# janelia-flyem/flypylib

Measured on AMD Instinct MI355X. Metric: inference Mvoxels/sec, vgg_like (rf 18, 22^3 coarse -> 88^3 per reference tile), synthetic EM uint8 volume, higher is better.
Workload: dtype f16s; 1 GPU; the 520^3 volume of BASELINE.json's metric (configs[0]'s substack size) per GPU: vgg_like inference, 520x520x520 synthetic uint8 volume, reference tile lattice 102^3 (pitch 88), u8 in / f32 out resident in HBM; tile_in=102, executor=vgg_split_f16, parallelism=z-slab tile sharding x1, no collective, device=AMD Radeon Graphics (gfx950:sramecc+:xnack-)

## Files before the change

flypylib_amd/csrc/vgg_plan.h:

```cpp
#pragma once
#include <algorithm>
#include <cstdint>
#include <vector>

struct VggSlab {
  int64_t VZ, VY, VX;
  int64_t fz_hi;
  int64_t cz_lo, cz_hi;
  int CY, CX;
  bool empty;
};

static inline VggSlab vgg_slab(const int64_t dims[3], const std::vector<int32_t> &origins_z,
                               int32_t out_sz_z, int32_t zb, int32_t ze, int off) {
  VggSlab s = {};
  s.VZ = dims[0] - 2 * off; s.VY = dims[1] - 2 * off; s.VX = dims[2] - 2 * off;
  s.empty = s.VZ <= 0 || s.VY <= 0 || s.VX <= 0 || zb >= ze;
  if (s.empty) return s;
  const int64_t fz_lo = (int64_t)origins_z[zb] - off;
  s.fz_hi = std::min<int64_t>((int64_t)origins_z[ze - 1] - off + out_sz_z, s.VZ);
  s.cz_lo = fz_lo / 4; s.cz_hi = (s.fz_hi + 3) / 4;
  s.CY = (int)((s.VY + 3) / 4); s.CX = (int)((s.VX + 3) / 4);
  return s;
}

struct VggPyramid {
  int P2, P1;
  explicit VggPyramid(int64_t C) : P2((int)C + 2), P1(2 * P2 + 2) {}
};
struct Vgg2Pyramid {
  int Q, T3, H;
  explicit Vgg2Pyramid(int64_t C) : Q((int)C + 2), T3(2 * Q + 2), H(T3 + 2) {}
};

static inline int64_t vgg_chunk_rows(int64_t budget_bytes, int64_t bytes_per_fine_row,
                                     int fixed_rows, int64_t span, int64_t cap = 0) {
  int64_t c = std::max<int64_t>(4, (budget_bytes / bytes_per_fine_row - fixed_rows) / 2);
  c = std::min<int64_t>(c, span);
  c = (c + 3) / 4 * 4;
  return cap ? std::min<int64_t>(c, cap) : c;
}

static inline int64_t vgg_split_max_p1_rows(int P1Y, int P1X, int tile_z) {
  return ((int64_t)1 << 32) / 16 / ((int64_t)P1Y * P1X) - (tile_z + 2);
}
static inline int64_t vgg_split_chunk_cap(int64_t max_rows) {
  return std::max<int64_t>(4, ((max_rows - VggPyramid(0).P1) / 2) / 4 * 4);
}

enum { MID_INTERIOR = 0, MID_XCOL = 1, MID_ZLAYER = 2 };

struct MidGeo {
  int BZ, BY, BX;
  int ZS;
  constexpr int TZ() const { return BZ + 2; }
  constexpr int TY() const { return BY + 2; }
  constexpr int TX() const { return BX + 2; }
  constexpr int slots() const { return (TZ() - 1) * ZS + TY() * TX(); }
  constexpr int slot(int tz, int ty, int tx) const { return tz * ZS + ty * TX() + tx; }
};
constexpr MidGeo mid_geo(int o) {
  return o == MID_XCOL ? MidGeo{8, 16, 4, 108} : o == MID_ZLAYER ? MidGeo{4, 8, 16, 182} : MidGeo{8, 4, 16, 118};
}

struct MidVox { int z, y, x; };
constexpr MidVox mid_voxel(int o, int wave, int sub, int c) {
  return o == MID_XCOL     ? MidVox{2 * (wave >> 1) + (sub >> 1), c, 2 * (wave & 1) + (sub & 1)}
         : o == MID_ZLAYER ? MidVox{2 * (wave >> 2) + (sub >> 1), 2 * (wave & 3) + (sub & 1), c}
                           : MidVox{2 * (wave >> 1) + (sub >> 1), 2 * (wave & 1) + (sub & 1), c};
}
constexpr MidVox mid_slot_voxel(const MidGeo &g, int s) {
  const int tz = s / g.ZS < g.TZ() ? s / g.ZS : g.TZ() - 1;
  const int rem = s - tz * g.ZS < g.TY() * g.TX() ? s - tz * g.ZS : g.TY() * g.TX() - 1;
  return MidVox{tz, rem / g.TX(), rem % g.TX()};
}
constexpr int mid_tap_slot(const MidGeo &g, int tap) { return g.slot(tap / 9, (tap / 3) % 3, tap % 3); }

struct MidWalk {
  int nbx, nby, nbz;
  int z0, x0;
  constexpr int64_t blocks() const { return (int64_t)nbx * nby * nbz; }
};
struct MidPlan { MidWalk w[3]; };

static inline MidPlan vgg_mid_plan(int Z, int Y, int X, bool reorient) {
  auto cdiv = [](int a, int b) { return (a + b - 1) / b; };
  const MidGeo gi = mid_geo(MID_INTERIOR), gx = mid_geo(MID_XCOL), gz = mid_geo(MID_ZLAYER);
  MidPlan p = {};
  MidWalk &in = p.w[MID_INTERIOR], &xc = p.w[MID_XCOL], &zl = p.w[MID_ZLAYER];
  in = MidWalk{cdiv(2 * X, gi.BX), cdiv(2 * Y, gi.BY), cdiv(2 * Z, gi.BZ), 0, 0};
  if (!reorient) return p;
  const int live_x = 2 * X % gi.BX, live_z = 2 * Z % gi.BZ;
  if (live_x) {
    const MidWalk c = {cdiv(live_x, gx.BX), cdiv(2 * Y, gx.BY), cdiv(2 * Z, gx.BZ), 0, (in.nbx - 1) * gi.BX};
    if (c.blocks() < (int64_t)in.nby * in.nbz) { xc = c; --in.nbx; }
  }
  if (live_z && in.nbx) {
    const MidWalk c = {in.nbx, cdiv(2 * Y, gz.BY), cdiv(live_z, gz.BZ), (in.nbz - 1) * gi.BZ, 0};
    if (c.blocks() < (int64_t)in.nbx * in.nby) { zl = c; --in.nbz; }
  }
  return p;
}
```

flypylib_amd/csrc/vgg_split.hip:

```cpp
#define FPL_F16 1
#include <algorithm>
#include <cmath>
#include <initializer_list>

#include "fast_paths.h"
#include "mfma_util.h"
#include "pack_weights.h"
#include "vgg_plan.h"
#include <type_traits>
#include "vgg_split_lds.h"
#include "vgg_tiles.h"

namespace {

constexpr int CH = 48;
constexpr int CHP = 24, NPASS = CH / CHP;
constexpr int LO_OFF = CHP * 2;
constexpr int PASS_BYTES = 2 * LO_OFF;
constexpr int VOX = NPASS * PASS_BYTES;
constexpr int KS = (27 * CHP + 31) / 32;
constexpr int KTAB = (KS + 4) / 4 * 4;
constexpr int KTAB_BYTES = 4 * KTAB * 4;
static_assert(CHP % 8 == 0, "a lane's 8 k-slots stay inside one tap");

// ... 696 lines not shown
    for (int b = 0; b < 3; ++b) {
      const f32x4 sh = *reinterpret_cast<const f32x4 *>(a.shift3 + zero + 16 * b + 4 * g);
#pragma unroll
      for (int sub = 0; sub < 4; ++sub) acc[sub][b] = sh;
    }
    x8::conv_block(smem, ktab + 8 * g, td, origin(cur), origin(has_next ? nxt : cur), part, a.w3, vb,
                   sub_off, wave, lane, acc);
    asm volatile("" : "+s"(zero));
    const h16x8 *w4p = a.w4 + zero;
    f32x4 sh4[3];
#pragma unroll
    for (int b = 0; b < 3; ++b)
#pragma unroll
      for (int r = 0; r < 4; ++r) sh4[b][r] = a.shift4[zero + x8::out_channel(b, g, r)];
    h16x8 w4[3][4];
#pragma unroll
    for (int s = 0; s < 4; ++s)
#pragma unroll
      for (int b = 0; b < 3; ++b) w4[b][s] = w4p[(s * 3 + b) * 64 + lane];
    f32x4 pooled[3] = {{0.f, 0.f, 0.f, 0.f}, {0.f, 0.f, 0.f, 0.f}, {0.f, 0.f, 0.f, 0.f}};
    unsigned ovf = 0u;
#pragma unroll
    for (int sub = 0; sub < 4; ++sub) {
      const Frag2 h0 = pack_relu_split(acc[sub][0], acc[sub][1], ovf);
      const h16x8 hx = pack_relu_split_x(acc[sub][2], ovf);
#pragma unroll
      for (int b = 0; b < 3; ++b) {
        const f32x4 a4 = chain48(w4[b], h0, hx, sh4[b]);
#pragma unroll
        for (int r = 0; r < 4; ++r) pooled[b][r] = __builtin_fmaxf(pooled[b][r], a4[r]);
      }
    }
#pragma unroll
    for (int b = 0; b < 3; ++b)
#pragma unroll
      for (int r = 0; r < 4; ++r)
        pooled[b][r] = __builtin_fmaxf(pooled[b][r], __shfl_xor(pooled[b][r], 1));
    const int pz = 4 * cur.bz + pzl, py = 2 * cur.by + pyl, px = 8 * cur.bx + (c >> 1);
    const bool inside = pz < a.p2.Z && py < a.p2.Y && px < a.p2.X;
    if ((c & 1) == 0 && inside)
      x8::store12(a.p2, a.p2.vox(pz, py, px), g, pooled, ovf);
    ovf_all = pk_max_i16(ovf_all, inside ? ovf : 0u);
    if (!has_next) break;
    cur = nxt;
  }
  ovf_commit(ovf_all, a.flag, FPL_RANGE_MID);
}

static_assert(mid_geo(MID_INTERIOR).BZ == x8::BZ && mid_geo(MID_INTERIOR).BY == x8::BY &&
              mid_geo(MID_INTERIOR).BX == x8::BX && mid_geo(MID_INTERIOR).ZS == x8::ZS, "vgg_plan.h describes x8's block");
struct MidEdgeArgs {
  MidXArgs m;
  int z0, x0;
};

template <int O>
__global__ __launch_bounds__(64 * x8::WAVES, 2) void vggs_mid_pool_edge(MidEdgeArgs e) {
  constexpr MidGeo G = mid_geo(O);
  const MidXArgs &a = e.m;
  unsigned *ktab = reinterpret_cast<unsigned *>(smem + 2 * x8::BUF);
  const int tid = threadIdx.x, lane = tid & 63;
  const int wave = __builtin_amdgcn_readfirstlane(tid >> 6);
  const int c = lane & 15, g = lane >> 4;
  x8::ktab_init_oriented<O>(ktab, tid);
  const x8::TileDma td = x8::tile_dma_init_oriented<O>(wave, lane, a.p1.Y, a.p1.XP, (unsigned)a.p1.part_bytes());
  const int S = (int)gridDim.x >> 3, nbricks = a.walk.bricks();
  const int group = (int)blockIdx.x & 7, slot = (int)blockIdx.x >> 3;
  x8::Cursor cur;
  if (!x8::cursor_first(a.walk, nbricks, group, slot, S, cur)) return;
  const int64_t part = a.p1.part_bytes();
  auto origin = [&](const x8::Cursor &q) {
    return a.p1.p + a.p1.vox(e.z0 + G.BZ * q.bz, G.BY * q.by, e.x0 + G.BX * q.bx) * 16;
  };
  const MidVox v0 = mid_voxel(O, wave, 0, c);
  const unsigned vb = (unsigned)(G.slot(v0.z, v0.y, v0.x) * 16);
  auto sub_off = [](int sub) -> unsigned {
    const MidVox d = mid_voxel(O, 0, sub, 0);
    return (unsigned)(mid_geo(O).slot(d.z, d.y, d.x) * 16);
  };
  unsigned ovf_all = 0u;
  x8::prime(smem, td, origin(cur), part, a.w3, wave, lane);
  for (;;) {
    x8::Cursor nxt = cur;
    const bool has_next = x8::cursor_next(a.walk, slot, S, nxt);
    int zero = 0;
    asm volatile("" : "+s"(zero));
    f32x4 acc[4][3];
#pragma unroll
    for (int b = 0; b < 3; ++b) {
      const f32x4 sh = *reinterpret_cast<const f32x4 *>(a.shift3 + zero + 16 * b + 4 * g);
#pragma unroll
      for (int sub = 0; sub < 4; ++sub) acc[sub][b] = sh;
    }
    x8::conv_block(smem, ktab + 8 * g, td, origin(cur), origin(has_next ? nxt : cur), part, a.w3, vb,
                   sub_off, wave, lane, acc);
    asm volatile("" : "+s"(zero));
    const h16x8 *w4p = a.w4 + zero;
    f32x4 sh4[3];
#pragma unroll
    for (int b = 0; b < 3; ++b)
#pragma unroll
      for (int r = 0; r < 4; ++r) sh4[b][r] = a.shift4[zero + x8::out_channel(b, g, r)];
    h16x8 w4[3][4];
#pragma unroll
    for (int s = 0; s < 4; ++s)
#pragma unroll
      for (int b = 0; b < 3; ++b) w4[b][s] = w4p[(s * 3 + b) * 64 + lane];
    f32x4 pooled[3] = {{0.f, 0.f, 0.f, 0.f}, {0.f, 0.f, 0.f, 0.f}, {0.f, 0.f, 0.f, 0.f}};
    unsigned ovf = 0u;
#pragma unroll
    for (int sub = 0; sub < 4; ++sub) {
      const Frag2 h0 = pack_relu_split(acc[sub][0], acc[sub][1], ovf);
      const h16x8 hx = pack_relu_split_x(acc[sub][2], ovf);
#pragma unroll
      for (int b = 0; b < 3; ++b) {
        const f32x4 a4 = chain48(w4[b], h0, hx, sh4[b]);
#pragma unroll
        for (int r = 0; r < 4; ++r) pooled[b][r] = __builtin_fmaxf(pooled[b][r], a4[r]);
      }
    }
#pragma unroll
    for (int b = 0; b < 3; ++b)
#pragma unroll
      for (int r = 0; r < 4; ++r)
        pooled[b][r] = __builtin_fmaxf(pooled[b][r], __shfl_xor(pooled[b][r], 1));
    const int pz = (e.z0 + G.BZ * cur.bz + v0.z) >> 1, py = (G.BY * cur.by + v0.y) >> 1,
              px = (e.x0 + G.BX * cur.bx + v0.x) >> 1;
    const bool inside = pz < a.p2.Z && py < a.p2.Y && px < a.p2.X;
    if ((c & 1) == 0 && inside)
      x8::store12(a.p2, a.p2.vox(pz, py, px), g, pooled, ovf);
    ovf_all = pk_max_i16(ovf_all, inside ? ovf : 0u);
    if (!has_next) break;
    cur = nxt;
  }
  ovf_commit(ovf_all, a.flag, FPL_RANGE_MID);
}

constexpr int T_W7 = 3 * 6, T_W8 = 3;
__device__ __forceinline__ void head_chain(const f32x4 (&acc)[4][3], const unsigned char *w6p,
                                           const unsigned char *w7p, const unsigned char *w8p, const float *sh6p,
                                           const float *sh7p, float bias8, int lane, unsigned &ovf, float (&logit)[4]) {
  const int c = lane & 15, g = lane >> 4;
  auto frag = [&](const unsigned char *w, int part_, int nfrag, int f) {
    return *reinterpret_cast<const h16x8 *>(w + ((size_t)(part_ * nfrag + f) * 64 + lane) * 16);
  };
#pragma unroll
  for (int sp = 0; sp < 2; ++sp) {
    Frag2 h5[2];
    h16x8 h5x[2];
#pragma unroll
    for (int q = 0; q < 2; ++q) {
      h5[q] = pack_relu_split(acc[2 * sp + q][0], acc[2 * sp + q][1], ovf);
      h5x[q] = pack_relu_split_x(acc[2 * sp + q][2], ovf);
    }
    Frag2 h6[2][3];
#pragma unroll
    for (int s = 0; s < 3; ++s) {
      f32x4 a6[2][2];
#pragma unroll
      for (int bb = 0; bb < 2; ++bb) {
        const int b = 2 * s + bb;
        f32x4 sh;
#pragma unroll
        for (int r = 0; r < 4; ++r) sh[r] = sh6p[16 * b + 4 * g + r];
        h16x8 w6[4];
#pragma unroll
        for (int t = 0; t < 4; ++t) w6[t] = frag(w6p, 0, 0, t * 6 + b);
#pragma unroll
        for (int q = 0; q < 2; ++q) a6[q][bb] = chain48(w6, h5[q], h5x[q], sh);
      }
#pragma unroll
      for (int q = 0; q < 2; ++q) h6[q][s] = pack_relu_split(a6[q][0], a6[q][1], ovf);
    }
    f32x4 a8[2] = {{0.f, 0.f, 0.f, 0.f}, {0.f, 0.f, 0.f, 0.f}};
#pragma unroll
    for (int s = 0; s < 3; ++s) {
      f32x4 a7[2][2];
#pragma unroll
      for (int bb = 0; bb < 2; ++bb) {
        const int b = 2 * s + bb;
        f32x4 sh;
#pragma unroll
        for (int r = 0; r < 4; ++r) sh[r] = sh7p[16 * b + 4 * g + r];
#pragma unroll
// ... 417 lines not shown
    const fpl_op &op = prog->ops[conv_ops[l]];
    std::vector<float> scale(A + op.scale_off, A + op.scale_off + op.cout);
    st->off_w[l] = all.size() * sizeof(uint16_t);
    if (l == 0 && v2) {
      fpl_pack_stem2_split(A + op.w_off, scale.data(), op.cout, NPASS, CHP, &all);
    } else if (l == 0) {
      for (int part = 0; part < 2; ++part) {
        std::vector<uint16_t> f;
        fpl_pack_stem(A + op.w_off, scale.data(), op.cout, &f, part);
        all.insert(all.end(), f.begin(), f.end());
      }
    } else if (op.k == 3 && !v2) {
      fpl_pack_passes_split(A + op.w_off, scale.data(), op.cin, op.cout, x8::NQ, x8::CQ, x8::KQ, 0, &all);
    } else if (op.k == 3) {
      fpl_pack_passes_split(A + op.w_off, scale.data(), op.cin, op.cout, NPASS, CHP, KS,
                            v2 && l >= 1 && l <= 3, &all);
    } else if (op.cin == CH) {
      static const int blk[4][2] = {{0, 1}, {0, 1}, {2, 2}, {2, 2}};
      static const int part[4][2] = {{0, 0}, {1, 1}, {1, 0}, {0, 1}};
      std::vector<uint16_t> f;
      for (int s = 0; s < 4; ++s)
        fpl_pack_chain_step(A + op.w_off, scale.data(), op.cin, op.cout, mblocks[l], blk[s], part[s], &f,
                            op.cout == CH ? 2 : 0);
      all.insert(all.end(), f.begin(), f.end());
    } else {
      for (int part = 0; part < 2; ++part) {
        std::vector<uint16_t> f;
        fpl_pack_frags(A + op.w_off, scale.data(), 1, op.cin, op.cout, mblocks[l], ksteps[l],
                       SLOT_CHAIN, &f, false, part);
        all.insert(all.end(), f.begin(), f.end());
      }
    }
    st->off_s[l] = fpl_append_shifts(&shifts, A + op.shift_off, op.cout);
  }
  if (fpl_any_half_nonfinite(all))
    return fpl_fail_range(ctx, "a folded weight exceeds the IEEE-half range (65504); use precision "
                               "f32 (or 'auto') for this network");
  {
    const fpl_op &op0 = prog->ops[0];
    std::vector<float> sh48(48, 0.f);
    memcpy(sh48.data(), A + op0.shift_off, op0.cout * sizeof(float));
    st->xlim = (float)stem_input_limit(A, op0, A + op0.scale_off, sh48.data(), 1);
    if (!(st->xlim > 0.f))
      return fpl_fail_range(ctx, "the first layer's shift exceeds the IEEE-half range; use precision f32 "
                                 "(or 'auto') for this network");
  }
  st->bias8 = A[prog->ops[9].shift_off];
  FPL_TRY(fpl_upload_weight_set(ctx, all, shifts, &st->frags, &st->shifts));
  FPL_HIP(ctx, hipFuncSetAttribute((const void *)vggs_stem_pool<uint8_t>,
                                   hipFuncAttributeMaxDynamicSharedMemorySize, S_SMEM));
  FPL_HIP(ctx, hipFuncSetAttribute((const void *)vggs_stem_pool<float>,
                                   hipFuncAttributeMaxDynamicSharedMemorySize, S_SMEM));
  FPL_HIP(ctx, hipFuncSetAttribute((const void *)vggs_mid_pool,
                                   hipFuncAttributeMaxDynamicSharedMemorySize, x8::SMEM));
  FPL_HIP(ctx, hipFuncSetAttribute((const void *)vggs_mid_pool_edge<MID_XCOL>,
                                   hipFuncAttributeMaxDynamicSharedMemorySize, x8::SMEM));
  FPL_HIP(ctx, hipFuncSetAttribute((const void *)vggs_mid_pool_edge<MID_ZLAYER>,
                                   hipFuncAttributeMaxDynamicSharedMemorySize, x8::SMEM));
  FPL_HIP(ctx, hipFuncSetAttribute((const void *)vggs_c5_tail_p24,
                                   hipFuncAttributeMaxDynamicSharedMemorySize, M_SMEM));
  FPL_HIP(ctx, hipFuncSetAttribute((const void *)vggs_c5_tail,
                                   hipFuncAttributeMaxDynamicSharedMemorySize, x8::SMEM));
  FPL_HIP(ctx, hipFuncSetAttribute((const void *)vggs2_conv3<true, true, uint8_t>,
                                   hipFuncAttributeMaxDynamicSharedMemorySize, V2_SMEM));
  FPL_HIP(ctx, hipFuncSetAttribute((const void *)vggs2_conv3<true, true, float>,
                                   hipFuncAttributeMaxDynamicSharedMemorySize, V2_SMEM));
  FPL_HIP(ctx, hipFuncSetAttribute((const void *)vggs2_conv3<false, false, uint8_t>,
                                   hipFuncAttributeMaxDynamicSharedMemorySize, V2_SMEM));
  FPL_HIP(ctx, hipFuncSetAttribute((const void *)vggs2_conv3<false, true, uint8_t>,
                                   hipFuncAttributeMaxDynamicSharedMemorySize, V2_SMEM));
  st->version = prog->arena_version;
  st->int_valid = false;
  return 0;
}

int split_prepare_int(fpl_ctx *ctx, fpl_program *prog, SplitState *st, float mean, float sd) {
  if (st->int_valid && st->int_mean == mean && st->int_sd == sd) return 0;
  const fpl_op &op = prog->ops[0];
  const float *A = prog->arena_host.data();
  const double c0 = std::min(255.0, std::max(0.0, std::nearbyint((double)mean)));
  std::vector<float> scale(op.cout);
  st->shift1_int_host.assign(S_SHTAB, 0.f);
  const double k = (c0 - (double)mean) / (double)sd;
  for (int co = 0; co < op.cout; ++co) {
    scale[co] = (float)((double)A[op.scale_off + co] / (double)sd);
    for (int pz = 0; pz < 4; ++pz)
      for (int py = 0; py < 4; ++py)
        for (int px = 0; px < 4; ++px) {
          double sum = 0.0;
          for (int dz = 0; dz < 3 - pz; ++dz)
            for (int dy = 0; dy < 3 - py; ++dy)
              for (int dx = 0; dx < 3 - px; ++dx)
                sum += (double)A[op.w_off + (size_t)((dz * 3 + dy) * 3 + dx) * op.cout + co];
          st->shift1_int_host[(size_t)((pz * 4 + py) * 4 + px) * 48 + co] =
              (float)((double)A[op.shift_off + co] + k * sum * (double)A[op.scale_off + co]);
        }
  }
  st->w1_int_host.clear();
  if (fpl_vgg_variant(prog) == 2) {
    fpl_pack_stem2_split(A + op.w_off, scale.data(), op.cout, NPASS, CHP, &st->w1_int_host);
    st->w1_int_host.resize((size_t)2 * 6 * 512, 0);
  } else {
    for (int part = 0; part < 2; ++part) {
      std::vector<uint16_t> f;
      fpl_pack_stem(A + op.w_off, scale.data(), op.cout, &f, part);
      st->w1_int_host.insert(st->w1_int_host.end(), f.begin(), f.end());
// ... 83 lines not shown
      a.out = (unsigned char *)l3v; a.OZ = pz.T3; a.OY = py.T3; a.OX = px.T3;
      a.flag = flag;
      a.bg = BlockGrid{(int)ceil_div64(px.T3, 16), (int)ceil_div64(py.T3, 4), (int)ceil_div64(pz.T3, 4)};
      TimedLaunch tl(ctx, "vggs2_conv3");
      vggs2_conv3<false, false, uint8_t><<<brick_grid_size(a.bg), 256, V2_SMEM, stream>>>(a);
    }
    {
      V2SArgs a = {};
      a.in = (const unsigned char *)l3v; a.IZ = pz.T3; a.IY = py.T3; a.IX = px.T3;
      a.w = F + st->off_w[3]; a.shift = S + st->off_s[3];
      a.out = (unsigned char *)qv; a.OZ = pz.Q; a.OY = py.Q; a.OX = px.Q;
      a.flag = flag;
      a.bg = BlockGrid{(int)ceil_div64(px.Q, 8), (int)ceil_div64(py.Q, 2), (int)ceil_div64(pz.Q, 2)};
      TimedLaunch tl(ctx, "vggs2_conv3_pool");
      vggs2_conv3<false, true, uint8_t><<<brick_grid_size(a.bg), 256, V2_SMEM, stream>>>(a);
    }
    {
      TailSArgs a;
      a.p2 = (const unsigned char *)qv; a.P2Z = pz.Q; a.P2Y = py.Q; a.P2X = px.Q;
      a.w5 = F + st->off_w[4]; a.shift5 = S + st->off_s[4];
      a.CZ = CZ; a.CY = s.CY; a.CX = s.CX;
      a.w6 = F + st->off_w[5]; a.w7 = F + st->off_w[6]; a.w8 = F + st->off_w[7];
      a.shift6 = S + st->off_s[5]; a.shift7 = S + st->off_s[6]; a.bias8 = st->bias8;
      a.dst = dst; a.DY = SY; a.DX = SX; a.gz0 = c0;
      a.VZ = s.fz_hi; a.VY = s.VY; a.VX = s.VX; a.off = OFF;
      a.flag = flag;
      a.bg = BlockGrid{(int)ceil_div64(s.CX, 16), (int)ceil_div64(s.CY, 4), (int)ceil_div64(CZ, 4)};
      TimedLaunch tl(ctx, "vggs_c5_tail");
      vggs_c5_tail_p24<<<brick_grid_size(a.bg), 256, M_SMEM, stream>>>(a);
    }
    FPL_HIP(ctx, hipGetLastError());
  }
  return 0;
}

}

int fpl_split_infer_volume(fpl_ctx *ctx, fpl_program *prog, const void *src, int src_dtype,
                           float mean, float sd, const int64_t dims[3],
                           const std::vector<int32_t> origins[3], const int32_t out_sz[3],
                           int32_t zb, int32_t ze, float *dst) {
  SplitState *st;
  FPL_TRY(split_prepare(ctx, prog, &st));
  if (src_dtype == FPL_U8) FPL_TRY(split_prepare_int(ctx, prog, st, mean, sd));
  if (fpl_vgg_variant(prog) == 2)
    return split2_infer(ctx, st, src, src_dtype, mean, sd, dims, origins, out_sz, zb, ze, dst);
  hipStream_t stream = ctx->stream;
  const int64_t SZ = dims[0], SY = dims[1], SX = dims[2];
  const VggSlab s = vgg_slab(dims, origins[0], out_sz[0], zb, ze, 7);
  if (s.empty) return 0;
  const VggPyramid py(s.CY), px(s.CX);
  const char *edge_env = getenv("FPL_VGG_EDGE_BLOCKS");
  const int edge_blocks = edge_env ? atoi(edge_env) != 0 : 1;
  FPL_REQUIRE(ctx, (int64_t)S_TZ * SY * SX < ((int64_t)1 << 31),
              "vgg split path: a %lld x %lld plane is too large for the stem's 31-bit row "
              "offsets", (long long)SY, (long long)SX);
  const int64_t max_rows = vgg_split_max_p1_rows(py.P1, px.P1, x8::TZ);
  FPL_REQUIRE(ctx, max_rows >= 14,
              "vgg split path: a %lld x %lld plane is too large for the tile loader's 32-bit "
              "offsets", (long long)SY, (long long)SX);
  const int64_t cz_chunk = vgg_chunk_rows(fpl_vgg_scratch_budget(FPL_VGG_SCRATCH_DEFAULT),
                                          (int64_t)py.P1 * px.P1 * VOX, VggPyramid(0).P1, s.cz_hi - s.cz_lo,
                                          vgg_split_chunk_cap(max_rows));
  const VggPyramid pz_max(cz_chunk);
  DevTemp tmp(ctx);
  unsigned *flag;
  FPL_TRY(fpl_range_flag(ctx, &flag));
  x8::Tensor p1 = {nullptr, pz_max.P1, py.P1, px.P1, px.P1}, p2 = {nullptr, pz_max.P2, py.P2, px.P2, px.P2};
  void *p1v, *p2v;
  FPL_TRY(tmp.alloc((size_t)(p1.bytes() + p1.slack_bytes()), &p1v));
  FPL_TRY(tmp.alloc((size_t)(p2.bytes() + p2.slack_bytes()), &p2v));
  void *dumpv;
  FPL_TRY(tmp.alloc(256, &dumpv));
  const unsigned pgrid = (unsigned)std::max(8, ctx->n_cu / 8 * 8);
  const unsigned char *F = st->frags;
  const float *S = st->shifts;
  for (int64_t c0 = s.cz_lo; c0 < s.cz_hi; c0 += cz_chunk) {
    const int CZ = (int)std::min<int64_t>(cz_chunk, s.cz_hi - c0);
    const VggPyramid pz(CZ);
    p1 = x8::Tensor{(unsigned char *)p1v, pz.P1, py.P1, px.P1, px.P1};
    p2 = x8::Tensor{(unsigned char *)p2v, pz.P2, py.P2, px.P2, px.P2};
    FPL_HIP(ctx, hipMemsetAsync(p1.p + p1.bytes(), 0, (size_t)p1.slack_bytes(), stream));
    FPL_HIP(ctx, hipMemsetAsync(p2.p + p2.bytes(), 0, (size_t)p2.slack_bytes(), stream));
    {
      StemSArgs a;
      a.src = src; a.SZ = SZ; a.SY = SY; a.SX = SX; a.mean = mean; a.sd = sd;
      a.p1z0 = 2 * c0;
      a.z_hi = std::min<int64_t>(SZ, 4 * (c0 + CZ) + 14);
      a.w1 = (const h16x8 *)(F + st->off_w[0]);
      a.w2 = (const h16x8 *)(F + st->off_w[1]);
      a.shift1 = S + st->off_s[0]; a.shift2 = S + st->off_s[1];
      a.c0 = 0.f; a.shtab = nullptr;
      if (src_dtype == FPL_U8) {
        a.w1 = (const h16x8 *)st->w1_int; a.shtab = st->shift1_int;
        a.c0 = st->int_c0;
      }
      a.p1 = p1;
      a.flag = flag; a.xlim = st->xlim; a.dump = (unsigned char *)dumpv;
      a.nbx = (int)ceil_div64(px.P1, S_PX); a.nby = (int)ceil_div64(py.P1, S_PY);
      a.nbz = (int)ceil_div64(pz.P1, S_PZ);
      a.trim = edge_blocks;
      const unsigned grid = (unsigned)std::min<int64_t>((int64_t)a.nbx * a.nby * a.nbz,
                                                        (int64_t)ctx->n_cu);
      TimedLaunch tl(ctx, "vggs_stem_pool");
      if (src_dtype == FPL_U8)
        vggs_stem_pool<uint8_t><<<grid, 64 * S_WAVES, S_SMEM, stream>>>(a);
      else
        vggs_stem_pool<float><<<grid, 64 * S_WAVES, S_SMEM, stream>>>(a);
    }
    {
      MidXArgs a;
      a.p1 = p1;
      a.w3 = F + st->off_w[2];
      a.w4 = (const h16x8 *)(F + st->off_w[3]);
      a.shift3 = S + st->off_s[2]; a.shift4 = S + st->off_s[3];
      a.p2 = p2;
      a.flag = flag;
      const MidPlan mp = vgg_mid_plan(pz.P2, py.P2, px.P2, edge_blocks != 0);
      auto walk_of = [&](int o) { return x8::Walk{mp.w[o].nbx, mp.w[o].nby, mp.w[o].nbz}; };
      TimedLaunch tl(ctx, "vggs_mid_pool");
      if (mp.w[MID_INTERIOR].blocks()) {
        a.walk = walk_of(MID_INTERIOR);
        vggs_mid_pool<<<pgrid, 64 * x8::WAVES, x8::SMEM, stream>>>(a);
      }
      for (int o : {MID_XCOL, MID_ZLAYER}) {
        if (!mp.w[o].blocks()) continue;
        MidEdgeArgs e = {a, mp.w[o].z0, mp.w[o].x0};
        e.m.walk = walk_of(o);
        const unsigned egrid = (unsigned)std::min<int64_t>(pgrid, (mp.w[o].blocks() + 7) / 8 * 8);
        if (o == MID_XCOL)
          vggs_mid_pool_edge<MID_XCOL><<<egrid, 64 * x8::WAVES, x8::SMEM, stream>>>(e);
        else
          vggs_mid_pool_edge<MID_ZLAYER><<<egrid, 64 * x8::WAVES, x8::SMEM, stream>>>(e);
      }
    }
    {
      TailXArgs a;
      a.p2 = p2;
      a.w5 = F + st->off_w[4]; a.shift5 = S + st->off_s[4];
      a.CZ = CZ; a.CY = s.CY; a.CX = s.CX;
      a.w6 = F + st->off_w[5]; a.w7 = F + st->off_w[6]; a.w8 = F + st->off_w[7];
      a.shift6 = S + st->off_s[5]; a.shift7 = S + st->off_s[6]; a.bias8 = st->bias8;
      a.dst = dst; a.DY = SY; a.DX = SX; a.gz0 = c0;
      a.VZ = s.fz_hi; a.VY = s.VY; a.VX = s.VX; a.off = 7;
      a.flag = flag;
      a.walk = x8::Walk{(int)ceil_div64(s.CX, 16), (int)ceil_div64(s.CY, 4), (int)ceil_div64(CZ, 8)};
      TimedLaunch tl(ctx, "vggs_c5_tail");
      vggs_c5_tail<<<pgrid, 64 * x8::WAVES, x8::SMEM, stream>>>(a);
    }
    FPL_HIP(ctx, hipGetLastError());
  }
  return 0;
}
```

flypylib_amd/csrc/vgg_split_lds.h:

```cpp
#pragma once
#include "mfma_util.h"
#include "vgg_plan.h"
#include "vgg_tiles.h"

namespace x8 {

constexpr int CQ = 8, NQ = 6;
constexpr int KQ = 7;
constexpr int BZ = 8, BY = 4, BX = 16;
constexpr int TZ = BZ + 2, TY = BY + 2, TX = BX + 2;
constexpr int ZS = 118;
constexpr int PLANE = (TZ - 1) * ZS + TY * TX;
constexpr int CHUNKS = (2 * PLANE + 63) / 64;
constexpr int TILE_BYTES = CHUNKS * 1024;
constexpr int WFRAGS = KQ * 6;
constexpr int WBYTES = WFRAGS * 1024;
constexpr int BUF = TILE_BYTES + WBYTES;
constexpr int KTAB_BYTES = 4 * 8 * 4;
constexpr int SMEM = 2 * BUF + KTAB_BYTES;
constexpr int WAVES = 8;
constexpr int TCH = (CHUNKS + WAVES - 1) / WAVES;
constexpr int WCH = (WFRAGS + WAVES - 1) / WAVES;
static_assert((ZS - 2 * TX - 2) % 16 == 0 && (TX - 2) % 16 == 0, "conflict-free tap offsets");
static_assert(SMEM <= 160 * 1024, "one workgroup per CU");
// ... 206 lines not shown
};
__device__ __forceinline__ bool cursor_first(const Walk &w, int , int group, int slot, int S, Cursor &c) {
  const int total = w.nbx * w.nby * w.nbz, per = (total + 7) / 8;
  c.i = group * per + slot;
  c.iend = (group + 1) * per < total ? (group + 1) * per : total;
  if (c.i >= c.iend) return false;
  walk_decode(w, c.i, c.bx, c.by, c.bz);
  return true;
}
__device__ __forceinline__ bool cursor_next(const Walk &w, int , int S, Cursor &c) {
  c.i += S;
  if (c.i >= c.iend) return false;
  walk_decode(w, c.i, c.bx, c.by, c.bz);
  return true;
}

__host__ __device__ constexpr int out_channel(int b, int g, int r) { return b < 2 ? 8 * g + 4 * b + r : 32 + 4 * g + r; }
__device__ __forceinline__ void store12(const Tensor &t, int64_t vox, int g, const f32x4 (&v)[3], unsigned &ovf) {
  unsigned hi[6], lo[6];
#pragma unroll
  for (int b = 0; b < 3; ++b) {
    const Pair2 p0 = split_pk(v[b][0], v[b][1], ovf), p1 = split_pk(v[b][2], v[b][3], ovf);
    hi[2 * b] = p0.hi; hi[2 * b + 1] = p1.hi;
    lo[2 * b] = p0.lo; lo[2 * b + 1] = p1.lo;
  }
  const int64_t part = t.part_bytes();
  unsigned char *q = t.p + (int64_t)g * 2 * part + vox * 16;
  unsigned char *h = t.p + (int64_t)(4 + (g >> 1)) * 2 * part + vox * 16 + 8 * (g & 1);
  *reinterpret_cast<u32x4 *>(q) = u32x4{hi[0], hi[1], hi[2], hi[3]};
  *reinterpret_cast<u32x4 *>(q + part) = u32x4{lo[0], lo[1], lo[2], lo[3]};
  *reinterpret_cast<u32x2 *>(h) = u32x2{hi[4], hi[5]};
  *reinterpret_cast<u32x2 *>(h + part) = u32x2{lo[4], lo[5]};
}

__device__ __forceinline__ void store12_sel(const Tensor &t, int64_t vox, int g, const f32x4 (&v)[3],
                                            unsigned &ovf, bool valid, unsigned char *dump) {
  unsigned hi[6], lo[6], o2 = 0u;
#pragma unroll
  for (int b = 0; b < 3; ++b) {
    const Pair2 p0 = split_pk(v[b][0], v[b][1], o2), p1 = split_pk(v[b][2], v[b][3], o2);
    hi[2 * b] = p0.hi; hi[2 * b + 1] = p1.hi;
    lo[2 * b] = p0.lo; lo[2 * b + 1] = p1.lo;
  }
  ovf_note(ovf, valid ? o2 : 0u);
  const int64_t part = t.part_bytes();
  unsigned char *q = t.p + (int64_t)g * 2 * part + vox * 16;
  unsigned char *h = t.p + (int64_t)(4 + (g >> 1)) * 2 * part + vox * 16 + 8 * (g & 1);
  *reinterpret_cast<u32x4 *>(valid ? q : dump) = u32x4{hi[0], hi[1], hi[2], hi[3]};
  *reinterpret_cast<u32x4 *>(valid ? q + part : dump + 16) = u32x4{lo[0], lo[1], lo[2], lo[3]};
  *reinterpret_cast<u32x2 *>(valid ? h : dump + 32) = u32x2{hi[4], hi[5]};
  *reinterpret_cast<u32x2 *>(valid ? h + part : dump + 48) = u32x2{lo[4], lo[5]};
}

}
```

Baseline: 16190 Mvoxels/s.

## Add 8x8x16 y-doubled mid-pool block kernel with single weight buffer

```diff
diff --git a/flypylib_amd/csrc/vgg_plan.h b/flypylib_amd/csrc/vgg_plan.h
--- a/flypylib_amd/csrc/vgg_plan.h
+++ b/flypylib_amd/csrc/vgg_plan.h
@@ -48,7 +48,7 @@
   return std::max<int64_t>(4, ((max_rows - VggPyramid(0).P1) / 2) / 4 * 4);
 }
 
-enum { MID_INTERIOR = 0, MID_XCOL = 1, MID_ZLAYER = 2 };
+enum { MID_INTERIOR = 0, MID_XCOL = 1, MID_ZLAYER = 2, MID_Y8 = 3 };
 
 struct MidGeo {
   int BZ, BY, BX;
@@ -60,13 +60,18 @@
   constexpr int slot(int tz, int ty, int tx) const { return tz * ZS + ty * TX() + tx; }
 };
 constexpr MidGeo mid_geo(int o) {
-  return o == MID_XCOL ? MidGeo{8, 16, 4, 108} : o == MID_ZLAYER ? MidGeo{4, 8, 16, 182} : MidGeo{8, 4, 16, 118};
+  return o == MID_XCOL     ? MidGeo{8, 16, 4, 108}
+         : o == MID_ZLAYER ? MidGeo{4, 8, 16, 182}
+         : o == MID_Y8     ? MidGeo{8, 8, 16, 182}
+                           : MidGeo{8, 4, 16, 118};
 }
+constexpr int mid_subs(int o) { return o == MID_Y8 ? 8 : 4; }
 
 struct MidVox { int z, y, x; };
 constexpr MidVox mid_voxel(int o, int wave, int sub, int c) {
   return o == MID_XCOL     ? MidVox{2 * (wave >> 1) + (sub >> 1), c, 2 * (wave & 1) + (sub & 1)}
          : o == MID_ZLAYER ? MidVox{2 * (wave >> 2) + (sub >> 1), 2 * (wave & 3) + (sub & 1), c}
+         : o == MID_Y8     ? MidVox{2 * (wave >> 1) + ((sub >> 1) & 1), 4 * (wave & 1) + 2 * (sub >> 2) + (sub & 1), c}
                            : MidVox{2 * (wave >> 1) + (sub >> 1), 2 * (wave & 1) + (sub & 1), c};
 }
 constexpr MidVox mid_slot_voxel(const MidGeo &g, int s) {
@@ -75,6 +80,10 @@
   return MidVox{tz, rem / g.TX(), rem % g.TX()};
 }
 constexpr int mid_tap_slot(const MidGeo &g, int tap) { return g.slot(tap / 9, (tap / 3) % 3, tap % 3); }
+
+constexpr int MID_Y8_CHUNKS = (2 * mid_geo(MID_Y8).slots() + 63) / 64;
+constexpr int MID_Y8_ROUNDS = (MID_Y8_CHUNKS + 7) / 8;
+constexpr int mid_y8_chunk(int wave, int i) { return wave + 8 * i < MID_Y8_CHUNKS ? wave + 8 * i : -1; }
 
 struct MidWalk {
   int nbx, nby, nbz;
@@ -101,3 +110,22 @@
   }
   return p;
 }
+
+struct MidPlanY8 {
+  MidPlan p;
+  MidWalk y8;
+  int strip_y0;
+};
+
+static inline MidPlanY8 vgg_mid_plan_y8(int Z, int Y, int X, bool reorient, bool large) {
+  MidPlanY8 q = {vgg_mid_plan(Z, Y, X, reorient), MidWalk{}, 0};
+  MidWalk &in = q.p.w[MID_INTERIOR];
+  const MidGeo gi = mid_geo(MID_INTERIOR), g8 = mid_geo(MID_Y8);
+  const int rows8 = Y % 4 == 3 ? Y / 4 + 1 : Y / 4;
+  if (!large || !rows8 || !in.blocks()) return q;
+  q.y8 = MidWalk{in.nbx, rows8, in.nbz, 0, 0};
+  q.strip_y0 = rows8 * g8.BY;
+  in.nby = (2 * Y - q.strip_y0 + gi.BY - 1) / gi.BY;
+  if (in.nby <= 0) in = MidWalk{};
+  return q;
+}
diff --git a/flypylib_amd/csrc/vgg_split.hip b/flypylib_amd/csrc/vgg_split.hip
--- a/flypylib_amd/csrc/vgg_split.hip
+++ b/flypylib_amd/csrc/vgg_split.hip
@@ -772,6 +772,7 @@
 struct MidEdgeArgs {
   MidXArgs m;
   int z0, x0;
+  int y0;
 };
 
 template <int O>
@@ -790,7 +791,7 @@
   if (!x8::cursor_first(a.walk, nbricks, group, slot, S, cur)) return;
   const int64_t part = a.p1.part_bytes();
   auto origin = [&](const x8::Cursor &q) {
-    return a.p1.p + a.p1.vox(e.z0 + G.BZ * q.bz, G.BY * q.by, e.x0 + G.BX * q.bx) * 16;
+    return a.p1.p + a.p1.vox(e.z0 + G.BZ * q.bz, e.y0 + G.BY * q.by, e.x0 + G.BX * q.bx) * 16;
   };
   const MidVox v0 = mid_voxel(O, wave, 0, c);
   const unsigned vb = (unsigned)(G.slot(v0.z, v0.y, v0.x) * 16);
@@ -844,12 +845,92 @@
 #pragma unroll
       for (int r = 0; r < 4; ++r)
         pooled[b][r] = __builtin_fmaxf(pooled[b][r], __shfl_xor(pooled[b][r], 1));
-    const int pz = (e.z0 + G.BZ * cur.bz + v0.z) >> 1, py = (G.BY * cur.by + v0.y) >> 1,
+    const int pz = (e.z0 + G.BZ * cur.bz + v0.z) >> 1, py = (e.y0 + G.BY * cur.by + v0.y) >> 1,
               px = (e.x0 + G.BX * cur.bx + v0.x) >> 1;
     const bool inside = pz < a.p2.Z && py < a.p2.Y && px < a.p2.X;
     if ((c & 1) == 0 && inside)
       x8::store12(a.p2, a.p2.vox(pz, py, px), g, pooled, ovf);
     ovf_all = pk_max_i16(ovf_all, inside ? ovf : 0u);
+    if (!has_next) break;
+    cur = nxt;
+  }
+  ovf_commit(ovf_all, a.flag, FPL_RANGE_MID);
+}
+
+__global__ __launch_bounds__(64 * x8::WAVES, 2) void vggs_mid_pool_y8(MidXArgs a) {
+  namespace y8 = x8::y8;
+  constexpr MidGeo G = y8::G;
+  unsigned *ktab = reinterpret_cast<unsigned *>(smem + y8::KTAB_OFF);
+  const int tid = threadIdx.x, lane = tid & 63;
+  const int wave = __builtin_amdgcn_readfirstlane(tid >> 6);
+  const int c = lane & 15, g = lane >> 4;
+  y8::ktab_init(ktab, tid);
+  const y8::TileDma td = y8::tile_dma_init(wave, lane, a.p1.Y, a.p1.XP, (unsigned)a.p1.part_bytes());
+  const int S = (int)gridDim.x >> 3, nbricks = a.walk.bricks();
+  const int group = (int)blockIdx.x & 7, slot = (int)blockIdx.x >> 3;
+  x8::Cursor cur;
+  if (!x8::cursor_first(a.walk, nbricks, group, slot, S, cur)) return;
+  const int64_t part = a.p1.part_bytes();
+  auto origin = [&](const x8::Cursor &q) {
+    return a.p1.p + a.p1.vox(G.BZ * q.bz, G.BY * q.by, G.BX * q.bx) * 16;
+  };
+  const MidVox v0 = mid_voxel(MID_Y8, wave, 0, c);
+  const unsigned vb = (unsigned)(G.slot(v0.z, v0.y, v0.x) * 16);
+  unsigned ovf_all = 0u;
+  y8::prime(smem, td, origin(cur), a.w3, wave, lane);
+  for (;;) {
+    x8::Cursor nxt = cur;
+    const bool has_next = x8::cursor_next(a.walk, slot, S, nxt);
+    int zero = 0;
+    asm volatile("" : "+s"(zero));
+    f32x4 acc[y8::SUBS][3];
+#pragma unroll
+    for (int b = 0; b < 3; ++b) {
+      const f32x4 sh = *reinterpret_cast<const f32x4 *>(a.shift3 + zero + 16 * b + 4 * g);
+#pragma unroll
+      for (int sub = 0; sub < y8::SUBS; ++sub) acc[sub][b] = sh;
+    }
+    y8::conv_block(smem, ktab + 8 * g, td, origin(cur), origin(has_next ? nxt : cur), part, a.w3, vb, wave, lane,
+                   acc);
+    asm volatile("" : "+s"(zero));
+    const h16x8 *w4p = a.w4 + zero;
+    f32x4 sh4[3];
+#pragma unroll
+    for (int b = 0; b < 3; ++b)
+#pragma unroll
+      for (int r = 0; r < 4; ++r) sh4[b][r] = a.shift4[zero + x8::out_channel(b, g, r)];
+    h16x8 w4[3][4];
+#pragma unroll
+    for (int s = 0; s < 4; ++s)
+#pragma unroll
+      for (int b = 0; b < 3; ++b) w4[b][s] = w4p[(s * 3 + b) * 64 + lane];
+#pragma unroll
+    for (int win = 0; win < y8::SUBS / 4; ++win) {
+      f32x4 pooled[3] = {{0.f, 0.f, 0.f, 0.f}, {0.f, 0.f, 0.f, 0.f}, {0.f, 0.f, 0.f, 0.f}};
+      unsigned ovf = 0u;
+#pragma unroll
+      for (int sub = 4 * win; sub < 4 * win + 4; ++sub) {
+        const Frag2 h0 = pack_relu_split(acc[sub][0], acc[sub][1], ovf);
+        const h16x8 hx = pack_relu_split_x(acc[sub][2], ovf);
+#pragma unroll
+        for (int b = 0; b < 3; ++b) {
+          const f32x4 a4 = chain48(w4[b], h0, hx, sh4[b]);
+#pragma unroll
+          for (int r = 0; r < 4; ++r) pooled[b][r] = __builtin_fmaxf(pooled[b][r], a4[r]);
+        }
+      }
+#pragma unroll
+      for (int b = 0; b < 3; ++b)
+#pragma unroll
+        for (int r = 0; r < 4; ++r)
+          pooled[b][r] = __builtin_fmaxf(pooled[b][r], __shfl_xor(pooled[b][r], 1));
+      const MidVox vw = mid_voxel(MID_Y8, wave, 4 * win, c);
+      const int pz = (G.BZ * cur.bz + vw.z) >> 1, py = (G.BY * cur.by + vw.y) >> 1, px = (G.BX * cur.bx + vw.x) >> 1;
+      const bool inside = pz < a.p2.Z && py < a.p2.Y && px < a.p2.X;
+      if ((c & 1) == 0 && inside)
+        x8::store12(a.p2, a.p2.vox(pz, py, px), g, pooled, ovf);
+      ovf_all = pk_max_i16(ovf_all, inside ? ovf : 0u);
+    }
     if (!has_next) break;
     cur = nxt;
   }
@@ -1373,6 +1454,10 @@
   FPL_HIP(ctx, hipFuncSetAttribute((const void *)vggs_stem_pool<float>,
                                    hipFuncAttributeMaxDynamicSharedMemorySize, S_SMEM));
   FPL_HIP(ctx, hipFuncSetAttribute((const void *)vggs_mid_pool,
+                                   hipFuncAttributeMaxDynamicSharedMemorySize, x8::SMEM));
+  FPL_HIP(ctx, hipFuncSetAttribute((const void *)vggs_mid_pool_y8,
+                                   hipFuncAttributeMaxDynamicSharedMemorySize, x8::y8::SMEM));
+  FPL_HIP(ctx, hipFuncSetAttribute((const void *)vggs_mid_pool_edge<MID_INTERIOR>,
                                    hipFuncAttributeMaxDynamicSharedMemorySize, x8::SMEM));
   FPL_HIP(ctx, hipFuncSetAttribute((const void *)vggs_mid_pool_edge<MID_XCOL>,
                                    hipFuncAttributeMaxDynamicSharedMemorySize, x8::SMEM));
@@ -1562,6 +1647,8 @@
   const VggPyramid py(s.CY), px(s.CX);
   const char *edge_env = getenv("FPL_VGG_EDGE_BLOCKS");
   const int edge_blocks = edge_env ? atoi(edge_env) != 0 : 1;
+  const char *mid_env = getenv("FPL_VGG_MID_BLOCK");
+  const int mid_large = mid_env ? atoi(mid_env) != 0 : 1;
   FPL_REQUIRE(ctx, (int64_t)S_TZ * SY * SX < ((int64_t)1 << 31),
               "vgg split path: a %lld x %lld plane is too large for the stem's 31-bit row "
               "offsets", (long long)SY, (long long)SX);
@@ -1626,19 +1713,27 @@
       a.shift3 = S + st->off_s[2]; a.shift4 = S + st->off_s[3];
       a.p2 = p2;
       a.flag = flag;
-      const MidPlan mp = vgg_mid_plan(pz.P2, py.P2, px.P2, edge_blocks != 0);
-      auto walk_of = [&](int o) { return x8::Walk{mp.w[o].nbx, mp.w[o].nby, mp.w[o].nbz}; };
+      const MidPlanY8 mq = vgg_mid_plan_y8(pz.P2, py.P2, px.P2, edge_blocks != 0, mid_large != 0);
+      const MidPlan &mp = mq.p;
+      auto walk_of = [&](const MidWalk &w) { return x8::Walk{w.nbx, w.nby, w.nbz}; };
+      auto grid_of = [&](const MidWalk &w) { return (unsigned)std::min<int64_t>(pgrid, (w.blocks() + 7) / 8 * 8); };
       TimedLaunch tl(ctx, "vggs_mid_pool");
-      if (mp.w[MID_INTERIOR].blocks()) {
-        a.walk = walk_of(MID_INTERIOR);
+      if (mq.y8.blocks()) {
+        a.walk = walk_of(mq.y8);
+        vggs_mid_pool_y8<<<grid_of(mq.y8), 64 * x8::WAVES, x8::y8::SMEM, stream>>>(a);
+      }
+      if (mp.w[MID_INTERIOR].blocks() && !mq.strip_y0) {
+        a.walk = walk_of(mp.w[MID_INTERIOR]);
         vggs_mid_pool<<<pgrid, 64 * x8::WAVES, x8::SMEM, stream>>>(a);
       }
-      for (int o : {MID_XCOL, MID_ZLAYER}) {
-        if (!mp.w[o].blocks()) continue;
-        MidEdgeArgs e = {a, mp.w[o].z0, mp.w[o].x0};
-        e.m.walk = walk_of(o);
-        const unsigned egrid = (unsigned)std::min<int64_t>(pgrid, (mp.w[o].blocks() + 7) / 8 * 8);
-        if (o == MID_XCOL)
+      for (int o : {MID_INTERIOR, MID_XCOL, MID_ZLAYER}) {
+        if (!mp.w[o].blocks() || (o == MID_INTERIOR && !mq.strip_y0)) continue;
+        MidEdgeArgs e = {a, mp.w[o].z0, mp.w[o].x0, o == MID_INTERIOR ? mq.strip_y0 : 0};
+        e.m.walk = walk_of(mp.w[o]);
+        const unsigned egrid = grid_of(mp.w[o]);
+        if (o == MID_INTERIOR)
+          vggs_mid_pool_edge<MID_INTERIOR><<<egrid, 64 * x8::WAVES, x8::SMEM, stream>>>(e);
+        else if (o == MID_XCOL)
           vggs_mid_pool_edge<MID_XCOL><<<egrid, 64 * x8::WAVES, x8::SMEM, stream>>>(e);
         else
           vggs_mid_pool_edge<MID_ZLAYER><<<egrid, 64 * x8::WAVES, x8::SMEM, stream>>>(e);
diff --git a/flypylib_amd/csrc/vgg_split_lds.h b/flypylib_amd/csrc/vgg_split_lds.h
--- a/flypylib_amd/csrc/vgg_split_lds.h
+++ b/flypylib_amd/csrc/vgg_split_lds.h
@@ -282,4 +282,202 @@
   *reinterpret_cast<u32x2 *>(valid ? h + part : dump + 48) = u32x2{lo[4], lo[5]};
 }
 
-}
+namespace y8 {
+
+constexpr MidGeo G = mid_geo(MID_Y8);
+constexpr int SUBS = mid_subs(MID_Y8);
+constexpr int PLANE = G.slots();
+constexpr int CHUNKS = MID_Y8_CHUNKS;
+constexpr int TCH = MID_Y8_ROUNDS;
+constexpr int TILE_BYTES = CHUNKS * 1024;
+constexpr int WA = 4 * 6, WB = WFRAGS - WA;
+constexpr int W_OFF = 2 * TILE_BYTES;
+constexpr int KTAB_OFF = W_OFF + WBYTES;
+constexpr int SMEM = KTAB_OFF + KTAB_BYTES;
+static_assert(G.BZ == 8 && G.BY == 8 && G.BX == 16 && SUBS * WAVES * 16 == G.BZ * G.BY * G.BX, "");
+static_assert((G.ZS - 2 * G.TX() - 2) % 16 == 0 && (G.TX() - 2) % 16 == 0, "conflict-free tap offsets");
+static_assert(PLANE == 1818 && CHUNKS == 57 && TCH == 8 && SMEM == 159872 && SMEM <= 160 * 1024, "LDS budget");
+static_assert(WA % WAVES == 0 && WB <= 3 * WAVES, "weight chunk deal");
+
+struct TileDma {
+  unsigned off[TCH];
+};
+__device__ __forceinline__ TileDma tile_dma_init(int wave, int lane, int SY, int SX, unsigned part_bytes) {
+  TileDma d;
+#pragma unroll
+  for (int i = 0; i < TCH; ++i) {
+    int slot = 64 * (wave + WAVES * i) + lane;
+    slot = slot < 2 * PLANE ? slot : 2 * PLANE - 1;
+    const int part = slot >= PLANE;
+    const MidVox v = mid_slot_voxel(G, slot - part * PLANE);
+    d.off[i] = (unsigned)(((v.z * SY + v.y) * SX + v.x) * 16) + (part ? part_bytes : 0u);
+  }
+  return d;
+}
+
+__device__ __forceinline__ void ktab_init(unsigned *ktab, int tid) {
+  if (tid < 32) {
+    const int g = tid >> 3, s = tid & 7;
+    const int tap = 4 * s + g;
+    ktab[tid] = tap < 27 ? (unsigned)(mid_tap_slot(G, tap) * 16) : 0u;
+  }
+}
+
+__device__ __forceinline__ void dma_tile(const TileDma &d, int i, int wave, const unsigned char *org, unsigned char *tile) {
+  const int j = wave + WAVES * i;
+  if (i < TCH - 1 || j < CHUNKS) {
+    asm volatile("" : "+s"(org));
+    glds16(org + d.off[i], tile + j * 1024);
+  }
+}
+__device__ __forceinline__ void dma_weights(int first, int n, int k, int wave, int lane, const unsigned char *wpass,
+                                            unsigned char *wbuf) {
+  const int j = wave + WAVES * k;
+  if (j < n) {
+    const unsigned char *src = wpass + (first + j) * 1024;
+    asm volatile("" : "+s"(src));
+    glds16(src + (unsigned)lane * 16u, wbuf + (first + j) * 1024);
+  }
+}
+
+__device__ __forceinline__ void dma_step(int s, const TileDma &d, int wave, int lane, const unsigned char *wcur,
+                                         const unsigned char *wnxt, const unsigned char *org, unsigned char *tile,
+                                         unsigned char *wbuf) {
+  if (s == 0) {
+#pragma unroll
+    for (int k = 0; k < 3; ++k) dma_weights(WA, WB, k, wave, lane, wcur, wbuf);
+  } else if (s == 1 || s == 2) {
+#pragma unroll
+    for (int k = 0; k < 3; ++k) dma_tile(d, 3 * (s - 1) + k, wave, org, tile);
+  } else if (s == 3) {
+    dma_tile(d, 6, wave, org, tile);
+    dma_tile(d, 7, wave, org, tile);
+    dma_weights(0, WA, 0, wave, lane, wnxt, wbuf);
+  } else if (s == 4) {
+    dma_weights(0, WA, 1, wave, lane, wnxt, wbuf);
+    dma_weights(0, WA, 2, wave, lane, wnxt, wbuf);
+  }
+}
+
+__device__ __forceinline__ constexpr unsigned sub_off(int sub) {
+  return (unsigned)(G.slot(mid_voxel(MID_Y8, 0, sub, 0).z, mid_voxel(MID_Y8, 0, sub, 0).y, 0) * 16);
+}
+
+template <typename Issue>
+__device__ __forceinline__ void pass_kloop(const unsigned char *tile, const unsigned char *wbuf, const unsigned *ktab_g,
+                                           unsigned vb, Issue issue, int lane, f32x4 (&acc)[SUBS][3]) {
+  const unsigned char *wl = wbuf + lane * 16;
+  const u32x4 k0 = *reinterpret_cast<const u32x4 *>(ktab_g), k1 = *reinterpret_cast<const u32x4 *>(ktab_g + 4);
+  Frag2 ba[4], bb[4];
+  h16x8 w[6];
+#pragma unroll
+  for (int q = 0; q < 4; ++q) {
+    const unsigned char *p = tile + vb + k0[0] + sub_off(q);
+    ba[q].hi = *reinterpret_cast<const h16x8 *>(p);
+    ba[q].lo = *reinterpret_cast<const h16x8 *>(p + PLANE * 16);
+  }
+#pragma unroll
+  for (int f = 0; f < 6; ++f) w[f] = *reinterpret_cast<const h16x8 *>(wl + f * 1024);
+#pragma unroll
+  for (int s = 0; s < KQ; ++s) {
+    const unsigned kcur = s < 4 ? k0[s & 3] : k1[s & 3];
+    __builtin_amdgcn_sched_barrier(0);
+    __builtin_amdgcn_s_setprio(1);
+#pragma unroll
+    for (int q = 0; q < 4; ++q)
+#pragma unroll
+      for (int b = 0; b < 3; ++b) acc[q][b] = mfma16(w[3 + b], ba[q].hi, acc[q][b]);
+    __builtin_amdgcn_sched_barrier(0);
+#pragma unroll
+    for (int q = 0; q < 4; ++q) {
+      const unsigned char *p = tile + vb + kcur + sub_off(4 + q);
+      bb[q].hi = *reinterpret_cast<const h16x8 *>(p);
+      bb[q].lo = *reinterpret_cast<const h16x8 *>(p + PLANE * 16);
+    }
+    __builtin_amdgcn_sched_barrier(0);
+#pragma unroll
+    for (int q = 0; q < 4; ++q)
+#pragma unroll
+      for (int b = 0; b < 3; ++b) acc[q][b] = mfma16(w[b], ba[q].lo, acc[q][b]);
+    __builtin_amdgcn_sched_barrier(0);
+    issue(s);
+    __builtin_amdgcn_sched_barrier(0);
+#pragma unroll
+    for (int q = 0; q < 4; ++q)
+#pragma unroll
+      for (int b = 0; b < 3; ++b) acc[q][b] = mfma16(w[b], ba[q].hi, acc[q][b]);
+#pragma unroll
+    for (int q = 0; q < 4; ++q)
+#pragma unroll
+      for (int b = 0; b < 3; ++b) acc[4 + q][b] = mfma16(w[3 + b], bb[q].hi, acc[4 + q][b]);
+    __builtin_amdgcn_sched_barrier(0);
+    if (s + 1 < KQ) {
+      const unsigned knxt = s + 1 < 4 ? k0[(s + 1) & 3] : k1[(s + 1) & 3];
+#pragma unroll
+      for (int q = 0; q < 4; ++q) {
+        const unsigned char *p = tile + vb + knxt + sub_off(q);
+        ba[q].hi = *reinterpret_cast<const h16x8 *>(p);
+        ba[q].lo = *reinterpret_cast<const h16x8 *>(p + PLANE * 16);
+      }
+#pragma unroll
+      for (int f = 3; f < 6; ++f) w[f] = *reinterpret_cast<const h16x8 *>(wl + ((s + 1) * 6 + f) * 1024);
+    }
+    __builtin_amdgcn_sched_barrier(0);
+#pragma unroll
+    for (int q = 0; q < 4; ++q)
+#pragma unroll
+      for (int b = 0; b < 3; ++b) acc[4 + q][b] = mfma16(w[b], bb[q].lo, acc[4 + q][b]);
+#pragma unroll
+    for (int q = 0; q < 4; ++q)
+#pragma unroll
+      for (int b = 0; b < 3; ++b) acc[4 + q][b] = mfma16(w[b], bb[q].hi, acc[4 + q][b]);
+    __builtin_amdgcn_s_setprio(0);
+    __builtin_amdgcn_sched_barrier(0);
+    if (s + 1 < KQ) {
+#pragma unroll
+      for (int f = 0; f < 3; ++f) w[f] = *reinterpret_cast<const h16x8 *>(wl + ((s + 1) * 6 + f) * 1024);
+    }
+  }
+}
+
+__device__ __forceinline__ void conv_block(unsigned char *smem, const unsigned *ktab_g, const TileDma &td,
+                                           const unsigned char *org_cur, const unsigned char *org_nxt,
+                                           int64_t part_bytes, const unsigned char *wglobal, unsigned vb, int wave,
+                                           int lane, f32x4 (&acc)[SUBS][3]) {
+  unsigned char *wbuf = smem + W_OFF;
+#pragma unroll 1
+  for (int pp = 0; pp < NQ / 2; ++pp) {
+#pragma unroll
+    for (int h = 0; h < 2; ++h) {
+      const int pass = 2 * pp + h;
+      unsigned char *tile = smem + h * TILE_BYTES, *other = smem + (h ^ 1) * TILE_BYTES;
+      const bool more = pass + 1 < NQ;
+      const unsigned char *torg = more ? org_cur + (int64_t)(pass + 1) * 2 * part_bytes : org_nxt;
+      const unsigned char *wcur = wglobal + (size_t)pass * WBYTES;
+      const unsigned char *wnxt = wglobal + (size_t)(more ? pass + 1 : 0) * WBYTES;
+      auto issue = [&](int s) {
+        if (s <= 4) {
+          __builtin_amdgcn_s_setprio(0);
+          if (s == 3) __syncthreads();
+          dma_step(s, td, wave, lane, wcur, wnxt, torg, other, wbuf);
+          __builtin_amdgcn_s_setprio(1);
+        }
+      };
+      pass_kloop(tile, wbuf, ktab_g, vb, issue, lane, acc);
+      __syncthreads();
+    }
+  }
+}
+
+__device__ __forceinline__ void prime(unsigned char *smem, const TileDma &td, const unsigned char *org,
+                                      const unsigned char *wglobal, int wave, int lane) {
+#pragma unroll
+  for (int i = 0; i < TCH; ++i) dma_tile(td, i, wave, org, smem);
+#pragma unroll
+  for (int k = 0; k < WA / WAVES; ++k) dma_weights(0, WA, k, wave, lane, wglobal, smem + W_OFF);
+  __syncthreads();
+}
+
+}
+
+}
```

Measured after the change: 16270 Mvoxels/s, median of 2. No clear change (+0.5%).
